# WPI-MMR/gym_solo

Measured on AMD Instinct MI355X. Metric: env-steps/s (whole node), 4096 Solo8 envs/GPU, 1/2/4/8 MI355X, higher is better.
Workload: dtype f64

## Files before the change

### gym_solo_amd/csrc/solo_engine.hip

```cpp
#include <hip/hip_runtime.h>

#include <cstdio>
#include <cstdlib>
#include <cstring>
#include <new>
#include <string>
#include <vector>

#include "solo_wave_ops.h"
#include "solo_pgs_gfx950.h"
#include "solo_step_kernel.h"
#include "solo_launch.h"

namespace solo_engine_detail {

struct EngineBase {
  virtual ~EngineBase() {}
  virtual int set_program(const SoloProgram* p) = 0;
  virtual int reset(const uint8_t* mask, hipStream_t s) = 0;
  virtual int settle(hipStream_t s) = 0;
  virtual int set_targets(const void* a, hipStream_t s) = 0;
  virtual int step(const void* a, uint32_t flags, hipStream_t s) = 0;
  virtual int rollout(const void* a, int k, uint32_t flags, void* obs_out, void* reward_out, void* done_out, hipStream_t s) = 0;
  virtual int view(SoloStateView* v) = 0;
  virtual int set_params(int which, const void* p, hipStream_t s) = 0;
  virtual int set_terrain(const SoloTerrain* t, hipStream_t s) = 0;
  virtual int set_order(const int32_t* order, hipStream_t s) = 0;
  virtual int time_step(const void* a, uint32_t flags, int reps, hipStream_t s, double* ms) = 0;
  virtual int time_rollout(const void* a, int k, uint32_t flags, void* obs_out, void* reward_out, void* done_out, hipStream_t s, double* ms) = 0;
  virtual int plan(int k, SoloLaunchPlan* out) = 0;
  virtual int reserve(int k, uint32_t flags) = 0;
  virtual int check_fault() = 0;
  virtual const char* kernel_name() = 0;
  virtual int set_control(const SoloControl* c, hipStream_t s) = 0;
  virtual int get_control(SoloControl* out) = 0;
  virtual int set_contact_sensing(int32_t enable, hipStream_t s) = 0;
  virtual int get_contacts(void** out) = 0;
  std::string err;
};

#define HIP_TRY(expr)                                                                 \
  do {                                                                                \
    hipError_t e_ = (expr);                                                           \
    if (e_ != hipSuccess) {                                                           \
      err = std::string(#expr) + ": " + hipGetErrorString(e_);                        \
      return SOLO_ERR_HIP;                                                            \
    }                                                                                 \
  } while (0)

constexpr size_t kStatsBytes = (size_t)SOLO_STATS_SHARDS * SOLO_STATS_WIDTH * sizeof(double);

template <typename T>
struct Engine final : EngineBase {
  SoloConfig cfg;
  SoloModel model;
  int n = 0, device = 0, obs_dim = 0;
  bool have_program = false;
  SoloControl control{};
  bool settling = false;
  solo::KParams<T> hparams;
  solo::KParams<T>* dparams = nullptr;
  T *state = nullptr, *snapshot = nullptr, *targets = nullptr, *params = nullptr, *obs = nullptr,
    *reward = nullptr, *settle_actions = nullptr, *warm = nullptr;
  T* traj = nullptr;
  uint8_t* done = nullptr;
  int32_t* term_count = nullptr;
  int32_t *order = nullptr, *cost = nullptr;
  bool use_order = false;
  double* stats = nullptr;
  T* terrain = nullptr;
  int32_t* queue = nullptr;
  size_t queue_ints = 0;
  int traj_steps = 0;
  int32_t* fault_host = nullptr;
  int32_t* fault_dev = nullptr;
  bool sensing = false;
  T *contact = nullptr, *contact_traj = nullptr;
#ifdef SOLO_STAMPS
  unsigned long long* stamps = nullptr;
#endif

  ~Engine() override {
    (void)hipSetDevice(device);
    for (int g = 0; g < kMaxStreams; ++g) {
      if (sub[g]) (void)hipStreamDestroy(sub[g]);
      if (ev_join[g]) (void)hipEventDestroy(ev_join[g]);
    }
    if (ev_fork) (void)hipEventDestroy(ev_fork);
    for (void* p : {(void*)dparams, (void*)state, (void*)snapshot, (void*)targets, (void*)params,
                    (void*)obs, (void*)reward, (void*)settle_actions, (void*)done,
                    (void*)term_count, (void*)order, (void*)cost, (void*)stats, (void*)terrain, (void*)traj, (void*)queue, (void*)warm, (void*)contact, (void*)contact_traj})
// ... 630 lines not shown
```

### gym_solo_amd/csrc/solo_step_kernel.h

```cpp
#pragma once

#include "solo_kernel_params.h"
#include "solo_outputs.h"

#if defined(SOLO_STAMPS) && defined(SOLO_STAMPS_LIGHT)
#define SOLO_STAMP(B, i)                                                                          \
  do {                                                                                            \
    if (((i) == 0 || (i) == 14) && solo::lane_id() == 0)                                          \
      (B).stamps[(size_t)(B).stamp_row * 32 + (i)] = __builtin_amdgcn_s_memrealtime();         \
  } while (0)
#elif defined(SOLO_STAMPS)
#ifdef SOLO_STAMPS_EPILOGUE
#define SOLO_STAMP_ON(i) ((i) == 0 || (i) >= 13)
#define SOLO_STAMP_E(B, i) SOLO_STAMP_AT(B, i)
#else
#define SOLO_STAMP_ON(i) true
#endif
#define SOLO_STAMP(B, i) do { if (SOLO_STAMP_ON(i)) SOLO_STAMP_AT(B, i); } while (0)
#define SOLO_STAMP_AT(B, i)                                                                       \
  do {                                                                                            \
    if (solo::lane_id() == 0) {                                                                   \
      const unsigned long long t_ = __builtin_amdgcn_s_memtime();                                 \
      (B).stamps[(size_t)(B).stamp_row * 32 + (i)] = t_;                                            \
      (B).acc[(i)] += t_ - (B).acc[16];                                                           \
      (B).acc[16] = t_;                                                                           \
    }                                                                                             \
  } while (0)
#else
#define SOLO_STAMP(B, i) do {} while (0)
#endif
#ifndef SOLO_STAMP_E
#define SOLO_STAMP_E(B, i) do {} while (0)
#endif

#ifndef SOLO_PGS_SWEEP_HOOK
#define SOLO_PGS_SWEEP_HOOK(it, pend, lam, v) do {} while (0)
#endif

namespace solo {

template <typename T> struct V3 { T x, y, z; };
template <typename T> __device__ __forceinline__ V3<T> operator+(V3<T> a, V3<T> b) { return {a.x + b.x, a.y + b.y, a.z + b.z}; }
template <typename T> __device__ __forceinline__ V3<T> operator-(V3<T> a, V3<T> b) { return {a.x - b.x, a.y - b.y, a.z - b.z}; }
template <typename T> __device__ __forceinline__ V3<T> operator*(T s, V3<T> a) { return {s * a.x, s * a.y, s * a.z}; }
template <typename T> __device__ __forceinline__ T dot(V3<T> a, V3<T> b) { return a.x * b.x + a.y * b.y + a.z * b.z; }
template <typename T> __device__ __forceinline__ V3<T> cross(V3<T> a, V3<T> b) {
  return {a.y * b.z - a.z * b.y, a.z * b.x - a.x * b.z, a.x * b.y - a.y * b.x};
}
template <typename T> __device__ __forceinline__ V3<T> roty(T c, T s, V3<T> v) {
  return {c * v.x + s * v.z, v.y, c * v.z - s * v.x};
}
template <typename T> __device__ __forceinline__ V3<T> ycross(V3<T> r) { return {r.z, T(0), -r.x}; }
template <typename T> __device__ __forceinline__ V3<T> symmul(const T* I, V3<T> v) {
  return {I[0] * v.x + I[3] * v.y + I[4] * v.z, I[3] * v.x + I[1] * v.y + I[5] * v.z,
          I[4] * v.x + I[5] * v.y + I[2] * v.z};
}
template <typename T> __device__ __forceinline__ void rot_inertia_y(T c, T s, const T* I, T* o) {
  const T cc = c * c, ss = s * s, cs = c * s;
  o[0] = cc * I[0] + T(2) * cs * I[4] + ss * I[2];
  o[1] = I[1];
  o[2] = ss * I[0] - T(2) * cs * I[4] + cc * I[2];
  o[3] = c * I[3] + s * I[5];
  o[4] = cs * (I[2] - I[0]) + (cc - ss) * I[4];
  o[5] = c * I[5] - s * I[3];
}
template <typename T> __device__ __forceinline__ T sum_over_group16(T x) { return wave_sum_group16(x); }
template <typename T> __device__ __forceinline__ V3<T> select(bool p, V3<T> a, V3<T> b) { return {p ? a.x : b.x, p ? a.y : b.y, p ? a.z : b.z}; }
template <typename T> __device__ __forceinline__ T both_halves(T x) { return x + wave_other_half16(x); }
template <typename T> __device__ __forceinline__ V3<T> both_halves(V3<T> v) { return {both_halves(v.x), both_halves(v.y), both_halves(v.z)}; }
template <typename T> __device__ __forceinline__ T from_lower(T x) { return wave_from_lower_half16(x); }
template <typename T> __device__ __forceinline__ V3<T> from_lower(V3<T> v) { return {from_lower(v.x), from_lower(v.y), from_lower(v.z)}; }


}
namespace solo {
#ifndef SOLO_PRIO_SWEEPS_F64
#define SOLO_PRIO_SWEEPS_F64 12
#endif
#ifndef SOLO_QUEUE_SPINS
#define SOLO_QUEUE_SPINS (1 << 22)
#endif
#ifndef SOLO_PRIO_BY_ROWS
#define SOLO_PRIO_BY_ROWS 1
#endif
#ifndef SOLO_PRIO_ROWS_1
#define SOLO_PRIO_ROWS_1 11
#define SOLO_PRIO_ROWS_2 17
#define SOLO_PRIO_ROWS_3 23
#endif
__device__ __forceinline__ int priority_by_rows(int rows) { return rows > SOLO_PRIO_ROWS_3 ? 3 : (rows > SOLO_PRIO_ROWS_2 ? 2 : (rows > SOLO_PRIO_ROWS_1 ? 1 : 0)); }
template <typename T> constexpr int kPrioSweeps = sizeof(T) == 4 ? 8 : SOLO_PRIO_SWEEPS_F64;
#ifndef SOLO_F64_WAVES
#define SOLO_F64_WAVES 4
#endif
template <typename T> constexpr int kRowBlockReals = sizeof(T) == 4 ? 64 * 8 + 64 * 8 : (SOLO_F64_WAVES >= 4 ? 800 : 896);
#ifndef SOLO_W4_PIPELINED_BUILD
#define SOLO_W4_PIPELINED_BUILD 0
#endif
#ifndef SOLO_W4_HYBRID_BUILD
#define SOLO_W4_HYBRID_BUILD 1
#endif
constexpr int kLegSlots = 26;

template <typename T> struct RowView {
  int type, body;
  const T* geo;
};
template <typename T> struct StepTables {
  const LegConst<T>* legc;
  const int32_t* rowtype;
  const T (*rowgeo)[4];
  __device__ __forceinline__ RowView<T> row(int lane) const {
    const int tb = rowtype[lane];
    return {tb & 15, (tb >> 4) & 15, rowgeo[(tb >> 8) & 255]};
  }
};

constexpr unsigned long long kPhaseLanes[3] = {0xc003c003c003c003ull,
                                               0x0924092409240924ull,
                                               0x36d836d836d836d8ull};

template <typename T, bool kResid, bool kFromLds>
__device__ __forceinline__ int pgs_solve_cpp(const ColumnBank<T>& A, T& v, T& lamv, T& cand, T& dl, unsigned long long& pend, T& lo, T& hi,
                                             T tol_rel, int lane, T mu, bool is_tan1, bool is_tangent, unsigned long long ph0,
                                             unsigned long long ph1, unsigned long long ph2, int iters, T diag, T resid_thr, int& n_changed) {
  using R = Real<T>;
  int it = 0;
#pragma unroll 1
  for (; it < iters && pend != 0ull; ++it) {
    const T lam_sweep_start = lamv;
    bool normals_moved = false;
#pragma unroll
    for (int phase = 0; phase < 3; ++phase) {
      const unsigned long long phase_lanes = phase == 0 ? ph0 : (phase == 1 ? ph1 : ph2);
      if (phase == 2 && normals_moved) {
        T n1, n2;
        if constexpr (ColumnBank<T>::kCompact) { n1 = wave_slot_below<1>(lamv); n2 = wave_slot_below<2>(lamv); }
        else { n1 = wave_lane_below<1>(lamv); n2 = wave_lane_below<2>(lamv); }
        const T lim = mu * (is_tan1 ? n1 : n2);
        lo = is_tangent ? -lim : lo;
        hi = is_tangent ? lim : hi;
        cand = R::clamp(v, lo, hi);
        dl = cand - lamv;
        pend = wave_ballot(R::abs(dl) > R::abs(lamv) * tol_rel);
      }
      if ((pend & phase_lanes) == 0ull) continue;
      if (phase == 1) normals_moved = true;
#pragma unroll
      for (int bank = 0; bank < (kFromLds ? 1 : ColumnBank<T>::kBanks); ++bank) {
        unsigned long long window = kFromLds ? phase_lanes : (phase_lanes & ColumnBank<T>::bank_lanes(bank));
#pragma unroll 1
        while ((pend & window) != 0ull) {
          const int r = __builtin_ctzll(pend & window);
          window &= ~((2ull << r) - 1ull);
          const T col = kFromLds ? A.column(r) : A.get(bank, r);
          const T delta = wave_readlane(dl, r);
          v = R::fma(col, delta, v);
          lamv = (lane == r) ? cand : lamv;
          cand = R::clamp(v, lo, hi);
          dl = cand - lamv;
          pend = wave_ballot(R::abs(dl) > R::abs(lamv) * tol_rel);
          ++n_changed;
        }
      }
    }
    SOLO_PGS_SWEEP_HOOK(it, pend, lamv, v);
    const T dvel = (lamv - lam_sweep_start) * diag;
    if (kResid && wave_ballot(dvel * dvel > resid_thr) == 0ull) { ++it; break; }
  }
  return it;
}

template <typename T, bool kResid, bool kPipelinedBuild, bool kCtl = false, bool kContact = false, typename FetchTarget>
__device__ __forceinline__ T physics_solve(const StepConst<T>& C, const KBuffers<T>& B, const StepTables<T>& tabs,
                                           const T* s_state, T my_target, FetchTarget&& fetch_target, T* s_rowvec, T (*s_hext)[8], unsigned char* s_rowleg,
                                           T* s_keep, T (*s_leg)[kLegSlots], const T* s_math, T mu, T mass_scale, int lane, int& row_at, bool& target_bad,
                                           int& prio_sweeps, int& prio_steps, int& prio_rot, T warm_in = T(0), bool warm_on = false,
                                           const CtlConst<T>* ctl = nullptr, T* s_cnrm = nullptr) {
  constexpr bool kCompact = ColumnBank<T>::kCompact;
  constexpr int kRS = ColumnBank<T>::kRowStride;
// ... 369 lines not shown
    hh[0] = jl1 * s_leg[leg][12];
    hh[1] = (jl2 - s_leg[leg][13] * hh[0]) * s_leg[leg][14];
  }
  T w = jl1 * s_leg[leg][15] + jl2 * s_leg[leg][16] - bias;
#pragma unroll
  for (int i = 0; i < 6; ++i) w += jb[i] * s_keep[21 + i];
  T diag = hh[0] * hh[0] + hh[1] * hh[1];
#pragma unroll
  for (int i = 0; i < 6; ++i) diag += gh[i] * gh[i];
  T inv_d = R::rcp(diag);
  if (!live) {
#pragma unroll
    for (int i = 0; i < 6; ++i) gh[i] = T(0);
    hh[0] = hh[1] = T(0);
    inv_d = T(0);
    w = T(0);
    diag = T(0);
  }
  T lam0 = T(0);
  if constexpr (kResid) {
    if (warm_on) {
      if constexpr (sizeof(T) == 8) mu = s_keep[27];
      const T imp0 = C.motor_impulse;
      lam0 = live ? C.warm_factor * warm_in : T(0);
      if (is_motor) lam0 = R::clamp(lam0, -imp0, imp0);
      else if (type == ROW_NORMAL || is_limit) lam0 = R::max(lam0, T(0));
      const T wn1 = wave_lane_below<1>(lam0), wn2 = wave_lane_below<2>(lam0);
      if (type == ROW_TAN1 || type == ROW_TAN2) {
        const T lim0 = (rc.body == BODY_BASE ? s_keep[29] : mu) * (type == ROW_TAN1 ? wn1 : wn2);
        lam0 = R::clamp(lam0, -lim0, lim0);
      }
      if (!live) lam0 = T(0);
      T zz[6], yy[2];
#pragma unroll
      for (int i = 0; i < 6; ++i) zz[i] = gh[i] * lam0;
      yy[0] = hh[0] * lam0;
      yy[1] = hh[1] * lam0;
      wave_reduce_rows(zz, yy);
      T alam = hh[0] * yy[0] + hh[1] * yy[1];
#pragma unroll
      for (int i = 0; i < 6; ++i) alam += gh[i] * zz[i];
      w += alam;
    }
  }
  const unsigned long long touching = wave_ballot(live && type == ROW_NORMAL);
  const unsigned long long limited = wave_ballot(live && is_limit);
  int sv_type = live ? type : (int)ROW_IDLE;
  T sv_v0 = w * -inv_d + lam0, sv_nid = -inv_d, sv_diag = diag;
  T sv_lam0 = lam0;
  T sv_imp = ctl_imp;
  T sg[6], sh[2];
  int sv_leg = leg, n_live = 64;
  bool sv_on_base = rc.body == BODY_BASE;
  if constexpr (!kCompact) {
#pragma unroll
    for (int i = 0; i < 6; ++i) { s_rowvec[lane * kRS + i] = gh[i]; sg[i] = gh[i]; }
    s_rowvec[lane * kRS + 6] = hh[0];
    s_rowvec[lane * kRS + 7] = hh[1];
    sh[0] = hh[0]; sh[1] = hh[1];
    s_hext[lane][2 * leg] = hh[0];
    s_hext[lane][2 * leg + 1] = hh[1];
    row_at = lane;
    wave_sync();
  } else {
    const unsigned long long live_lanes = wave_ballot(live);
    n_live = __builtin_popcountll(live_lanes);
    const int below = wave_count_below(live_lanes);
    const int dst = live ? below : n_live + (lane - below);
    row_at = dst;
#pragma unroll
    for (int i = 0; i < 6; ++i) s_rowvec[dst * kRS + i] = gh[i];
    s_rowvec[dst * kRS + 6] = hh[0];
    s_rowvec[dst * kRS + 7] = hh[1];
    s_rowleg[dst] = (unsigned char)leg;
    const int tl = wave_push_int(sv_type | (leg << 4) | (sv_on_base ? 64 : 0), dst);
    sv_v0 = wave_push(sv_v0, dst);
    sv_nid = wave_push(sv_nid, dst);
    if constexpr (kResid) { sv_diag = wave_push(sv_diag, dst); if (warm_on) sv_lam0 = wave_push(sv_lam0, dst); }
    if constexpr (kCtl) sv_imp = wave_push(sv_imp, dst);
    sv_type = tl & 15;
    sv_leg = (tl >> 4) & 3;
    sv_on_base = (tl & 64) != 0;
    wave_sync();
#pragma unroll
    for (int i = 0; i < 6; ++i) sg[i] = s_rowvec[lane * kRS + i];
    sh[0] = s_rowvec[lane * kRS + 6];
    sh[1] = s_rowvec[lane * kRS + 7];
  }

  SOLO_STAMP(B, 7);
#if SOLO_PRIO_BY_ROWS
  {
    const int rows_now = kCompact ? n_live : __builtin_popcountll(wave_ballot(live));
    wave_set_priority_level(prio_sweeps > kPrioSweeps<T> * prio_steps ? 3 : priority_by_rows(rows_now));
  }
#endif
  ColumnBank<T> A;
  if constexpr (kCompact) A.init(sg, sh, sv_nid, lane, s_rowvec, s_rowleg, sv_leg);
  else A.init(sg, sh, sv_nid, lane, s_rowvec, &s_hext[0][2 * sv_leg]);
  const bool overflow = kCompact && n_live > ColumnBank<T>::kSlots;
  if constexpr (!kCompact) {
#pragma unroll
    for (int l2 = 0; l2 < 4; ++l2) {
#pragma unroll
      for (int kk = 0; kk < 2; ++kk) A.build(16 * l2 + kk);
    }
    const unsigned touching_lo = (unsigned)touching, touching_hi = (unsigned)(touching >> 32);
    if (limited != 0ull) {
#pragma unroll
      for (int l2 = 0; l2 < 4; ++l2) {
#pragma unroll
        for (int kk = 14; kk < 16; ++kk)
          if ((limited >> (16 * l2 + kk)) & 1ull) A.build(16 * l2 + kk);
      }
    }
#pragma unroll
    for (int l2 = 0; l2 < 4; ++l2) {
#pragma unroll
      for (int j = 0; j < 4; ++j) {
        const int r0 = 16 * l2 + 2 + 3 * j;
        if (((r0 < 32 ? touching_lo : touching_hi) >> (r0 & 31)) & 1u) {
#pragma unroll
          for (int q = 0; q < 3; ++q) A.build(r0 + q);
        }
      }
    }
  } else if (!overflow) {
    if constexpr (SOLO_F64_WAVES >= 4 && SOLO_W4_HYBRID_BUILD && kPipelinedBuild) {
      typename ColumnBank<T>::Row cur = A.fetch(0);
      {
        typename ColumnBank<T>::Row nxt = A.fetch(1);
        A.build_from(0, cur);
        cur = A.fetch(2);
        A.build_from(1, nxt);
      }
#pragma unroll
      for (int j = 2; j < ColumnBank<T>::kSlots; j += 3) {
        if (n_live > j) {
          if (j + 2 < 17) {
            typename ColumnBank<T>::Row nxt = A.fetch(j + 1);
            A.build_from(j, cur);
            cur = A.fetch(j + 2);
            A.build_from(j + 1, nxt);
            nxt = A.fetch(j + 3);
            A.build_from(j + 2, cur);
            cur = nxt;
          } else {
            if (j == 17) A.build_from(j, cur); else A.build(j);
            if (j + 1 < ColumnBank<T>::kSlots) A.build(j + 1);
            if (j + 2 < ColumnBank<T>::kSlots) A.build(j + 2);
          }
        }
      }
    } else if constexpr (SOLO_F64_WAVES >= 4 && !SOLO_W4_PIPELINED_BUILD) {
      A.build(0); A.build(1);
#pragma unroll
      for (int j = 2; j < ColumnBank<T>::kSlots; j += 3) {
        if (n_live > j) {
          A.build(j);
          if (j + 1 < ColumnBank<T>::kSlots) A.build(j + 1);
          if (j + 2 < ColumnBank<T>::kSlots) A.build(j + 2);
        }
      }
    } else {
    typename ColumnBank<T>::Row cur = A.fetch(0);
    {
      const typename ColumnBank<T>::Row n1 = A.fetch(1);
      A.build_from(0, cur);
      cur = A.fetch(2);
      A.build_from(1, n1);
    }
#pragma unroll
    for (int j = 2; j < ColumnBank<T>::kSlots; j += 3) {
      if (n_live > j) {
        const typename ColumnBank<T>::Row n1 = A.fetch(j + 1 < 64 ? j + 1 : 63);
        A.build_from(j, cur);
        if (j + 1 < ColumnBank<T>::kSlots) {
          const typename ColumnBank<T>::Row n2 = A.fetch(j + 2 < 64 ? j + 2 : 63);
          A.build_from(j + 1, n1);
          cur = A.fetch(j + 3 < 64 ? j + 3 : 63);
          if (j + 2 < ColumnBank<T>::kSlots) A.build_from(j + 2, n2);
        }
      }
    }
    }
  }
  (void)touching; (void)limited;
  SOLO_STAMP(B, 8);
  const bool sv_motor = sv_type == ROW_MOTOR, sv_limit = sv_type == ROW_LIMIT, sv_normal = sv_type == ROW_NORMAL;
  const bool is_tan1 = sv_type == ROW_TAN1, is_tangent = sv_type == ROW_TAN1 || sv_type == ROW_TAN2;
  const T imp = C.motor_impulse;
  if constexpr (sizeof(T) == 8) mu = s_keep[27];
  mu = sv_on_base ? s_keep[29] : mu;
  T lo = T(0), hi = T(0);
  if (sv_motor) { lo = kCtl ? sv_imp : -imp; hi = kCtl ? sv_imp : imp; }
  else if (sv_normal || sv_limit) hi = R::big();
  T lamv = sv_lam0;
  T v = sv_v0;
  if constexpr (kResid) {
    if (warm_on) {
      T n1, n2;
      if constexpr (kCompact) { n1 = wave_slot_below<1>(lamv); n2 = wave_slot_below<2>(lamv); }
      else { n1 = wave_lane_below<1>(lamv); n2 = wave_lane_below<2>(lamv); }
      const T lim = mu * (is_tan1 ? n1 : n2);
      lo = is_tangent ? -lim : lo;
      hi = is_tangent ? lim : hi;
    }
  }
  const T tol_rel = T(wave_uniform(C.ulp_tol)) * R::half_ulp();
  const int iters = wave_uniform(C.iterations);
  const T resid_thr = C.resid_thr;
  unsigned long long ph0 = kPhaseLanes[0], ph1 = kPhaseLanes[1], ph2 = kPhaseLanes[2];
  if constexpr (kCompact) {
    ph0 = wave_ballot(sv_motor || sv_limit);
    ph1 = wave_ballot(sv_normal);
    ph2 = wave_ballot(is_tangent);
  }
  T cand = R::clamp(v, lo, hi);
  T dl = cand - lamv;
  unsigned long long pend = wave_ballot(R::abs(dl) > R::abs(lamv) * tol_rel);
  int n_changed = 0;
  int it = 0;
#ifdef SOLO_PGS_GFX950
  if (!overflow) {
    const unsigned long long tan1_lanes = wave_ballot(is_tan1), tangent_lanes = wave_ballot(is_tangent);
    if constexpr (!kResid) {
      it = pgs_solve_gfx950(A, v, lamv, cand, dl, pend, lo, hi, tol_rel, lane, mu, tan1_lanes, tangent_lanes, ph0, ph1, ph2, iters, n_changed);
    } else {
#pragma unroll 1
      for (;;) {
        const T lam_sweep_start = lamv;
        const int n = pgs_solve_gfx950(A, v, lamv, cand, dl, pend, lo, hi, tol_rel, lane, mu, tan1_lanes, tangent_lanes, ph0, ph1, ph2, 1, n_changed);
        it += n;
        if (n == 0 || it >= iters) break;
        const T dvel = (lamv - lam_sweep_start) * sv_diag;
        if (wave_ballot(dvel * dvel > resid_thr) == 0ull) break;
      }
    }
#if defined(SOLO_PGS_HAZARD_PROBE)
    {
      const unsigned stuck = __builtin_amdgcn_s_getreg((0 << 11) | (27 << 6) | 1);
      asm volatile("s_set_gpr_idx_off\n\ts_nop 1");
      if (stuck != 0 && lane == 0) stats_add(&B.stats[7], 1.0);
    }
#endif
  } else
#else
  if (!overflow) it = pgs_solve_cpp<T, kResid, false>(A, v, lamv, cand, dl, pend, lo, hi, tol_rel, lane, mu, is_tan1, is_tangent, ph0, ph1, ph2, iters, sv_diag, resid_thr, n_changed);
  else
#endif
  {
    if constexpr (kCompact) it = pgs_solve_cpp<T, kResid, true>(A, v, lamv, cand, dl, pend, lo, hi, tol_rel, lane, mu, is_tan1, is_tangent, ph0, ph1, ph2, iters, sv_diag, resid_thr, n_changed);
  }
#ifdef SOLO_STAMPS
  if (lane == 0) {
    const unsigned long long hw = (unsigned long long)(__builtin_amdgcn_s_getreg(63492) & 0xfffff), xcc = (unsigned long long)(__builtin_amdgcn_s_getreg(63508) & 0xf);
    B.stamps[(size_t)B.stamp_row * 32 + 15] = (unsigned long long)(it & 0xffff) | ((unsigned long long)__builtin_popcountll(touching) << 16) | (xcc << 24) | (hw << 28) | ((unsigned long long)(n_changed & 0xffff) << 48);
#ifndef SOLO_STAMPS_LIGHT
    B.acc[15] += (unsigned long long)it;
    B.acc[0] += (unsigned long long)n_changed;
#endif
  }
#endif
  (void)n_changed;
  if constexpr (kCompact) lamv = wave_pull(lamv, row_at);
  prio_sweeps += it;
  prio_steps += 1;
  prio_rot = prio_rot == 2 ? 0 : prio_rot + 1;
// ... 170 lines not shown
```

### gym_solo_amd/csrc/solo_wave_ops.h

```cpp
#pragma once

#include <hip/hip_runtime.h>

namespace solo {

__device__ __forceinline__ int lane_id() { return threadIdx.x; }
__device__ __forceinline__ int block_id() { return blockIdx.x; }

__device__ __forceinline__ void wave_sync() { __syncthreads(); }
__device__ __forceinline__ void wave_fence_global() {
  __builtin_amdgcn_fence(__ATOMIC_RELEASE, "workgroup");
  __builtin_amdgcn_fence(__ATOMIC_ACQUIRE, "workgroup");
}
template <typename P> __device__ __forceinline__ P* wave_opaque(P* p) {
  asm volatile("" : "+s"(p));
  return p;
}
__device__ __forceinline__ unsigned long long wave_opaque_bits(unsigned long long x) {
  asm volatile("" : "+s"(x));
  return x;
}
__device__ __forceinline__ int wave_opaque_lane(int lane) {
  asm volatile("" : "+v"(lane));
  return lane;
}
__device__ __forceinline__ int wave_fresh_lane() {
  int lane;
  asm volatile("v_mbcnt_lo_u32_b32 %0, -1, 0\n\tv_mbcnt_hi_u32_b32 %0, -1, %0" : "=v"(lane));
  return lane;
}
__device__ __forceinline__ int wave_readlane_int(int x, int lane) { return __builtin_amdgcn_readlane(x, lane); }
__device__ __forceinline__ int wave_uniform(int x) { return __builtin_amdgcn_readfirstlane(x); }

__device__ __forceinline__ float wave_readlane(float x, int lane) {
  return __int_as_float(__builtin_amdgcn_readlane(__float_as_int(x), lane));
}
__device__ __forceinline__ double wave_readlane(double x, int lane) {
  const long long b = __double_as_longlong(x);
  const int lo = __builtin_amdgcn_readlane((int)(b & 0xffffffffll), lane);
  const int hi = __builtin_amdgcn_readlane((int)(b >> 32), lane);
  return __longlong_as_double(((long long)hi << 32) | (unsigned int)lo);
}
__device__ __forceinline__ float wave_sum_legs(float x) {
  auto a = __builtin_amdgcn_permlane16_swap(__float_as_uint(x), __float_as_uint(x), false, false);
  const float s = __uint_as_float(a[0]) + __uint_as_float(a[1]);
  auto b = __builtin_amdgcn_permlane32_swap(__float_as_uint(s), __float_as_uint(s), false, false);
  return __uint_as_float(b[0]) + __uint_as_float(b[1]);
}
__device__ __forceinline__ double wave_sum_legs(double x) {
  unsigned lo = (unsigned)(__double_as_longlong(x) & 0xffffffffll), hi = (unsigned)(__double_as_longlong(x) >> 32);
  auto a = __builtin_amdgcn_permlane16_swap(lo, lo, false, false);
  auto b = __builtin_amdgcn_permlane16_swap(hi, hi, false, false);
  const double s = __longlong_as_double(((long long)a[0] & 0xffffffffll) | ((long long)b[0] << 32)) +
                   __longlong_as_double(((long long)a[1] & 0xffffffffll) | ((long long)b[1] << 32));
  lo = (unsigned)(__double_as_longlong(s) & 0xffffffffll); hi = (unsigned)(__double_as_longlong(s) >> 32);
  auto c = __builtin_amdgcn_permlane32_swap(lo, lo, false, false);
  auto d = __builtin_amdgcn_permlane32_swap(hi, hi, false, false);
  return __longlong_as_double(((long long)c[0] & 0xffffffffll) | ((long long)d[0] << 32)) +
         __longlong_as_double(((long long)c[1] & 0xffffffffll) | ((long long)d[1] << 32));
}
template <int CTRL> __device__ __forceinline__ float dpp_mov(float x) {
  return __int_as_float(__builtin_amdgcn_update_dpp(0, __float_as_int(x), CTRL, 0xf, 0xf, true));
}
template <int CTRL> __device__ __forceinline__ double dpp_mov(double x) {
  const long long b = __double_as_longlong(x);
  const int lo = __builtin_amdgcn_update_dpp(0, (int)(b & 0xffffffffll), CTRL, 0xf, 0xf, false);
  const int hi = __builtin_amdgcn_update_dpp(0, (int)(b >> 32), CTRL, 0xf, 0xf, false);
  return __longlong_as_double(((long long)hi << 32) | (unsigned int)lo);
}
template <typename T> __device__ __forceinline__ T wave_other_half16(T x) { return dpp_mov<0x128>(x); }
template <int BANKS> __device__ __forceinline__ float dpp_half_bcast(float x) {
  return __int_as_float(__builtin_amdgcn_update_dpp(__float_as_int(x), __float_as_int(x), 0x128, 0xf, BANKS, false));
}
template <int BANKS> __device__ __forceinline__ double dpp_half_bcast(double x) {
  const long long b = __double_as_longlong(x);
  const int lo = __builtin_amdgcn_update_dpp((int)(b & 0xffffffffll), (int)(b & 0xffffffffll), 0x128, 0xf, BANKS, false);
  const int hi = __builtin_amdgcn_update_dpp((int)(b >> 32), (int)(b >> 32), 0x128, 0xf, BANKS, false);
  return __longlong_as_double(((long long)hi << 32) | (unsigned int)lo);
}
template <typename T> __device__ __forceinline__ T wave_from_lower_half16(T x) { return dpp_half_bcast<0x3>(x); }
template <typename T> __device__ __forceinline__ T wave_from_upper_half16(T x) { return dpp_half_bcast<0xc>(x); }
template <int N, typename T> __device__ __forceinline__ T wave_lane_below(T x) { return dpp_mov<0x110 + N>(x); }
template <int N, typename T> __device__ __forceinline__ T wave_slot_below(T x) {
#pragma unroll
  for (int i = 0; i < N; ++i) x = dpp_mov<0x138>(x);
  return x;
}
__device__ __forceinline__ int wave_count_below(unsigned long long mask) {
  return (int)__builtin_amdgcn_mbcnt_hi((unsigned)(mask >> 32), __builtin_amdgcn_mbcnt_lo((unsigned)mask, 0u));
}
__device__ __forceinline__ int wave_push_int(int x, int dst) { return __builtin_amdgcn_ds_permute(dst << 2, x); }
__device__ __forceinline__ float wave_push(float x, int dst) { return __int_as_float(__builtin_amdgcn_ds_permute(dst << 2, __float_as_int(x))); }
__device__ __forceinline__ double wave_push(double x, int dst) {
  const long long b = __double_as_longlong(x);
  const int lo = __builtin_amdgcn_ds_permute(dst << 2, (int)(b & 0xffffffffll));
  const int hi = __builtin_amdgcn_ds_permute(dst << 2, (int)(b >> 32));
  return __longlong_as_double(((long long)hi << 32) | (unsigned int)lo);
}
__device__ __forceinline__ float wave_pull(float x, int src) { return __int_as_float(__builtin_amdgcn_ds_bpermute(src << 2, __float_as_int(x))); }
__device__ __forceinline__ double wave_pull(double x, int src) {
  const long long b = __double_as_longlong(x);
  const int lo = __builtin_amdgcn_ds_bpermute(src << 2, (int)(b & 0xffffffffll));
  const int hi = __builtin_amdgcn_ds_bpermute(src << 2, (int)(b >> 32));
  return __longlong_as_double(((long long)hi << 32) | (unsigned int)lo);
}
template <typename T> __device__ __forceinline__ T wave_sum_group16(T x) {
  x += dpp_mov<0x128>(x);
  x += dpp_mov<0x124>(x);
  x += dpp_mov<0x122>(x);
  x += dpp_mov<0x121>(x);
  return x;
}
__device__ __forceinline__ float wave_sum_all(float x) {
  x = wave_sum_group16(x);
  asm("s_nop 1\n\tv_add_f32_dpp %0, %0, %0 row_bcast:15 row_mask:0xa bank_mask:0xf\n\t"
      "s_nop 1\n\tv_add_f32_dpp %0, %0, %0 row_bcast:31 row_mask:0xc bank_mask:0xf" : "+v"(x));
  return wave_readlane(x, 63);
}
__device__ __forceinline__ double wave_sum_all(double x) { return wave_sum_legs(wave_sum_group16(x)); }
__device__ __forceinline__ unsigned long long wave_ballot(bool p) { return __ballot(p); }

__device__ __forceinline__ void wave_reduce_rows(float (&z)[6], float (&y)[2]) {
#define SOLO_DPP_STAGE8(CTRL)                                                                      \
  "v_add_f32_dpp %0, %0, %0 " CTRL " row_mask:0xf bank_mask:0xf\n\t"                                \
  "v_add_f32_dpp %1, %1, %1 " CTRL " row_mask:0xf bank_mask:0xf\n\t"                                \
  "v_add_f32_dpp %2, %2, %2 " CTRL " row_mask:0xf bank_mask:0xf\n\t"                                \
  "v_add_f32_dpp %3, %3, %3 " CTRL " row_mask:0xf bank_mask:0xf\n\t"                                \
  "v_add_f32_dpp %4, %4, %4 " CTRL " row_mask:0xf bank_mask:0xf\n\t"                                \
  "v_add_f32_dpp %5, %5, %5 " CTRL " row_mask:0xf bank_mask:0xf\n\t"                                \
  "v_add_f32_dpp %6, %6, %6 " CTRL " row_mask:0xf bank_mask:0xf\n\t"                                \
  "v_add_f32_dpp %7, %7, %7 " CTRL " row_mask:0xf bank_mask:0xf\n\t"
#define SOLO_DPP_STAGE6(CTRL, MASK)                                                                \
  "v_add_f32_dpp %0, %0, %0 " CTRL " row_mask:" MASK " bank_mask:0xf\n\t"                           \
  "v_add_f32_dpp %1, %1, %1 " CTRL " row_mask:" MASK " bank_mask:0xf\n\t"                           \
  "v_add_f32_dpp %2, %2, %2 " CTRL " row_mask:" MASK " bank_mask:0xf\n\t"                           \
  "v_add_f32_dpp %3, %3, %3 " CTRL " row_mask:" MASK " bank_mask:0xf\n\t"                           \
  "v_add_f32_dpp %4, %4, %4 " CTRL " row_mask:" MASK " bank_mask:0xf\n\t"                           \
  "v_add_f32_dpp %5, %5, %5 " CTRL " row_mask:" MASK " bank_mask:0xf\n\t"
  asm("s_nop 1\n\t"
      SOLO_DPP_STAGE8("row_ror:8") SOLO_DPP_STAGE8("row_ror:4") SOLO_DPP_STAGE8("row_ror:2") SOLO_DPP_STAGE8("row_ror:1")
      SOLO_DPP_STAGE6("row_bcast:15", "0xa") SOLO_DPP_STAGE6("row_bcast:31", "0xc")
      : "+v"(z[0]), "+v"(z[1]), "+v"(z[2]), "+v"(z[3]), "+v"(z[4]), "+v"(z[5]), "+v"(y[0]), "+v"(y[1]));
// ... 49 lines not shown
  __device__ __forceinline__ T dot(const T* rg, const T* rh, T same) const {
    const T a1 = __builtin_fma(g[2], rg[2], __builtin_fma(g[1], rg[1], g[0] * rg[0]));
    const T a2 = __builtin_fma(g[5], rg[5], __builtin_fma(g[4], rg[4], g[3] * rg[3]));
    return __builtin_fma(same, __builtin_fma(h[1], rh[1], h[0] * rh[0]), a1 + a2);
  }
};
template <> struct RowDot<float> {
  solo_f32x2 g01, g23, g45, h01;
  __device__ __forceinline__ void set(const float* gh, const float* hh) {
    g01 = solo_f32x2{gh[0], gh[1]}; g23 = solo_f32x2{gh[2], gh[3]}; g45 = solo_f32x2{gh[4], gh[5]};
    h01 = solo_f32x2{hh[0], hh[1]};
  }
  __device__ __forceinline__ float dot(const float* rg, const float* rh) const {
    const solo_f32x2* r = reinterpret_cast<const solo_f32x2*>(rg);
    solo_f32x2 acc = g01 * r[0];
    acc = g23 * r[1] + acc;
    acc = g45 * r[2] + acc;
    acc = h01 * *reinterpret_cast<const solo_f32x2*>(rh) + acc;
    return acc.x + acc.y;
  }
};

typedef float solo_f32x32 __attribute__((ext_vector_type(32)));
template <typename T> struct ColumnBank;
template <> struct ColumnBank<float> {
  static constexpr bool kResident = true;
  static constexpr bool kCompact = false;
  static constexpr int kSlots = 64, kRowStride = 8;
  static constexpr int kBanks = 2;
  static __device__ __forceinline__ constexpr unsigned long long bank_lanes(int b) { return 0xffffffffull << (32 * b); }
  RowDot<float> own;
  float nid;
  int lane;
  const float* rowvec;
  const float* hext;
  solo_f32x32 a0, a1;
  __device__ __forceinline__ void init(const float* gh, const float* hh, float nid_, int lane_, const float* rowvec_, const float* hext_) {
    own.set(gh, hh); nid = nid_; lane = lane_; rowvec = rowvec_; hext = hext_;
  }
  __device__ __forceinline__ float column(int r) const { const float m = (lane == r) ? 0.0f : nid; return m * own.dot(rowvec + 8 * r, hext + 8 * r); }
  __device__ __forceinline__ void build(int r) { const float x = column(r); if (r < 32) a0[r] = x; else a1[r - 32] = x; }
  __device__ __forceinline__ float get(int bank, int r) const { return bank == 0 ? a0[r & 31] : a1[r & 31]; }
};
typedef double solo_f64x16 __attribute__((ext_vector_type(16)));
template <> struct ColumnBank<double> {
  static constexpr bool kResident = true;
  static constexpr bool kCompact = true;
  static constexpr int kSlots = 32, kRowStride = 8;
  static constexpr int kBanks = 2;
  static __device__ __forceinline__ constexpr unsigned long long bank_lanes(int b) { return 0xffffull << (16 * b); }
  RowDot<double> own;
  double nid;
  int lane;
  const double* rowvec;
  const unsigned char* rowleg;
  int leg;
  solo_f64x16 a0, a1;
  __device__ __forceinline__ void init(const double* gh, const double* hh, double nid_, int lane_, const double* rowvec_, const unsigned char* rowleg_, int leg_) {
    own.set(gh, hh); nid = nid_; lane = lane_; rowvec = rowvec_; rowleg = rowleg_; leg = leg_;
  }
  __device__ __forceinline__ double same_leg(int leg_r) const { return leg_r == leg ? 1.0 : 0.0; }
  __device__ __forceinline__ double column(int r) const {
    const double m = (lane == r) ? 0.0 : nid;
    return m * own.dot(rowvec + kRowStride * r, rowvec + kRowStride * r + 6, same_leg(rowleg[r]));
  }
  __device__ __forceinline__ void build(int r) {
    const double x = column(r);
    if (r < 16) a0[r] = x; else a1[r - 16] = x;
  }
  struct Row { double g[6], h[2]; int leg; };
  __device__ __forceinline__ Row fetch(int r) const {
    Row x;
#pragma unroll
    for (int i = 0; i < 6; ++i) x.g[i] = rowvec[kRowStride * r + i];
    x.h[0] = rowvec[kRowStride * r + 6]; x.h[1] = rowvec[kRowStride * r + 7];
    x.leg = rowleg[r];
    return x;
  }
  __device__ __forceinline__ void build_from(int r, const Row& x) {
    const double m = (lane == r) ? 0.0 : nid;
    const double c = m * own.dot(x.g, x.h, same_leg(x.leg));
    if (r < 16) a0[r] = c; else a1[r - 16] = c;
  }
  __device__ __forceinline__ double get(int bank, int r) const { return bank == 0 ? a0[r & 15] : a1[r & 15]; }
};

template <typename B> using ColdArgs = const __attribute__((address_space(4))) B*;
template <typename B> __device__ __forceinline__ ColdArgs<B> wave_cold_args(const B& by_value) {
  (void)by_value;
  auto base = (const __attribute__((address_space(4))) char*)__builtin_amdgcn_kernarg_segment_ptr();
  ColdArgs<B> p = (ColdArgs<B>)(base + sizeof(void*));
  asm volatile("" : "+s"(p));
  return p;
}

__device__ __forceinline__ int wave_atomic_add(int32_t* p, int v) { return __hip_atomic_fetch_add(p, v, __ATOMIC_RELAXED, __HIP_MEMORY_SCOPE_AGENT); }
__device__ __forceinline__ int wave_atomic_load(const int32_t* p) { return __hip_atomic_load(p, __ATOMIC_RELAXED, __HIP_MEMORY_SCOPE_AGENT); }
__device__ __forceinline__ void wave_atomic_store(int32_t* p, int v) { __hip_atomic_store(p, v, __ATOMIC_RELAXED, __HIP_MEMORY_SCOPE_AGENT); }
__device__ __forceinline__ float wave_load_shared(const float* p) { return __uint_as_float(__hip_atomic_load(reinterpret_cast<const unsigned*>(p), __ATOMIC_RELAXED, __HIP_MEMORY_SCOPE_AGENT)); }
__device__ __forceinline__ double wave_load_shared(const double* p) { return __longlong_as_double((long long)__hip_atomic_load(reinterpret_cast<const unsigned long long*>(p), __ATOMIC_RELAXED, __HIP_MEMORY_SCOPE_AGENT)); }
__device__ __forceinline__ void wave_store_shared(float* p, float v) { __hip_atomic_store(reinterpret_cast<unsigned*>(p), __float_as_uint(v), __ATOMIC_RELAXED, __HIP_MEMORY_SCOPE_AGENT); }
__device__ __forceinline__ void wave_store_shared(double* p, double v) { __hip_atomic_store(reinterpret_cast<unsigned long long*>(p), (unsigned long long)__double_as_longlong(v), __ATOMIC_RELAXED, __HIP_MEMORY_SCOPE_AGENT); }
__device__ __forceinline__ void wave_release_device() {
  __builtin_amdgcn_fence(__ATOMIC_RELEASE, "workgroup");
  asm volatile("s_waitcnt vmcnt(0)" ::: "memory");
}
__device__ __forceinline__ void wave_acquire_device() { __builtin_amdgcn_fence(__ATOMIC_ACQUIRE, "workgroup"); }
__device__ __forceinline__ void wave_backoff() { __builtin_amdgcn_s_sleep(8); }
__device__ __forceinline__ void wave_fault_set(int32_t* p) { __hip_atomic_store(p, 1, __ATOMIC_RELAXED, __HIP_MEMORY_SCOPE_SYSTEM); }
__device__ __forceinline__ int wave_xcc_id() { return (int)(__builtin_amdgcn_s_getreg((3 << 11) | 20) & 0xf); }

__device__ __forceinline__ int wave_slot_id() { return (int)(__builtin_amdgcn_s_getreg(((4 - 1) << 11) | 4) & 0xf); }
__device__ __forceinline__ void wave_set_priority_level(int p) {
  if (p >= 3) __builtin_amdgcn_s_setprio(3);
  else if (p == 2) __builtin_amdgcn_s_setprio(2);
  else if (p == 1) __builtin_amdgcn_s_setprio(1);
  else __builtin_amdgcn_s_setprio(0);
}

template <typename T> struct Real;
template <> struct Real<float> {
  static __device__ __forceinline__ float sqrt(float x) { return __builtin_amdgcn_sqrtf(x); }
  static __device__ __forceinline__ float rsqrt(float x) { return __builtin_amdgcn_rsqf(x); }
  static __device__ __forceinline__ float rcp(float x) { return __builtin_amdgcn_rcpf(x); }
  static constexpr int kTabSize = 0;
  static __device__ __forceinline__ void sincos(float x, float* s, float* c, const float* = nullptr) {
    const float k = __builtin_rintf(x * 0.63661977236758134f);
    float r = __builtin_fmaf(k, -1.57079601287841796875f, x);
    r = __builtin_fmaf(k, -3.1391647326017846e-07f, r);
    r = __builtin_fmaf(k, -5.3903029534742385e-15f, r);
    const float r2 = r * r;
    float sp = __builtin_fmaf(r2, -1.9515295891e-4f, 8.3321608736e-3f);
    sp = __builtin_fmaf(r2, sp, -1.6666654611e-1f);
    const float sn = __builtin_fmaf(r2 * r, sp, r);
    float cp = __builtin_fmaf(r2, 2.443315711809948e-5f, -1.388731625493765e-3f);
    cp = __builtin_fmaf(r2, cp, 4.166664568298827e-2f);
    const float cs = __builtin_fmaf(r2 * r2, cp, __builtin_fmaf(r2, -0.5f, 1.0f));
    const int q = (int)k;
    const float a = (q & 1) ? cs : sn, b = (q & 1) ? sn : cs;
    *s = (q & 2) ? -a : a;
    *c = ((q + 1) & 2) ? -b : b;
  }
  static __device__ __forceinline__ void sinc_cos(float x2, float* sinc, float* c, const float* = nullptr) {
    if (__builtin_expect(__builtin_amdgcn_readfirstlane(__float_as_int(x2)) > 0x3d800000, 0)) {
      const float x = __builtin_amdgcn_sqrtf(x2);
      float sn, cs;
      sincos(x, &sn, &cs);
      *sinc = sn * __builtin_amdgcn_rcpf(x);
      *c = cs;
      return;
    }
    float sp = __builtin_fmaf(x2, -1.9841270e-4f, 8.3333333e-3f);
    sp = __builtin_fmaf(x2, sp, -1.6666667e-1f);
    *sinc = __builtin_fmaf(x2, sp, 1.0f);
    float cp = __builtin_fmaf(x2, 2.4801587e-5f, -1.3888889e-3f);
    cp = __builtin_fmaf(x2, cp, 4.1666667e-2f);
    cp = __builtin_fmaf(x2, cp, -0.5f);
    *c = __builtin_fmaf(x2, cp, 1.0f);
  }
  static __device__ __forceinline__ float atan2(float y, float x) {
    const float ax = fabsf(x), ay = fabsf(y);
    const float mx = fmaxf(ax, ay), mn = fminf(ax, ay);
    const float a = (mx == 0.0f) ? 0.0f : mn * __builtin_amdgcn_rcpf(mx);
    const float s2 = a * a;
    float p = __builtin_fmaf(s2, -0.0040545654f, 0.021862952f);
    p = __builtin_fmaf(s2, p, -0.05591232f);
// ... 139 lines not shown
```

Before: 190.8 million.

## Build f64 column bank two rows at a time using both wave halves

When the live contact rows fit in the column bank, each 32-lane half of the wave now computes a different row's dot products. The two results are exchanged with permlane32_swap, so each build step fills two column entries. Lanes in the upper half take over the lower half's row data (nid, leg and own row vector), so both halves cover the same 32 rows. The aim is to halve the number of serial f64 dot-product steps in the build phase. The cost is extra cross-lane swaps and a replacement of the pipelined fetch/build schedule. Correctness depends on live rows being at most 32 and on the upper half's lanes holding no needed state.

```diff
diff --git a/gym_solo_amd/csrc/solo_engine.hip b/gym_solo_amd/csrc/solo_engine.hip
--- a/gym_solo_amd/csrc/solo_engine.hip
+++ b/gym_solo_amd/csrc/solo_engine.hip
@@ -7,6 +7,9 @@
 #include <string>
 #include <vector>
 
+#ifndef SOLO_F64_PAIR_BUILD
+#define SOLO_F64_PAIR_BUILD 1
+#endif
 #include "solo_wave_ops.h"
 #include "solo_pgs_gfx950.h"
 #include "solo_step_kernel.h"
diff --git a/gym_solo_amd/csrc/solo_step_kernel.h b/gym_solo_amd/csrc/solo_step_kernel.h
--- a/gym_solo_amd/csrc/solo_step_kernel.h
+++ b/gym_solo_amd/csrc/solo_step_kernel.h
@@ -96,6 +96,9 @@
 template <typename T> constexpr int kRowBlockReals = sizeof(T) == 4 ? 64 * 8 + 64 * 8 : (SOLO_F64_WAVES >= 4 ? 800 : 896);
 #ifndef SOLO_W4_PIPELINED_BUILD
 #define SOLO_W4_PIPELINED_BUILD 0
+#endif
+#ifndef SOLO_F64_PAIR_BUILD
+#define SOLO_F64_PAIR_BUILD 0
 #endif
 #ifndef SOLO_W4_HYBRID_BUILD
 #define SOLO_W4_HYBRID_BUILD 1
@@ -631,10 +634,18 @@
     sv_leg = (tl >> 4) & 3;
     sv_on_base = (tl & 64) != 0;
     wave_sync();
-#pragma unroll
-    for (int i = 0; i < 6; ++i) sg[i] = s_rowvec[lane * kRS + i];
-    sh[0] = s_rowvec[lane * kRS + 6];
-    sh[1] = s_rowvec[lane * kRS + 7];
+    int own_slot = lane;
+#if SOLO_F64_PAIR_BUILD
+    if (n_live <= ColumnBank<T>::kSlots) {
+      own_slot = lane & 31;
+      sv_nid = wave_from_lower_half32(sv_nid);
+      sv_leg = (wave_from_lower_half32(tl) >> 4) & 3;
+    }
+#endif
+#pragma unroll
+    for (int i = 0; i < 6; ++i) sg[i] = s_rowvec[own_slot * kRS + i];
+    sh[0] = s_rowvec[own_slot * kRS + 6];
+    sh[1] = s_rowvec[own_slot * kRS + 7];
   }
 
   SOLO_STAMP(B, 7);
@@ -675,6 +686,16 @@
       }
     }
   } else if (!overflow) {
+#if SOLO_F64_PAIR_BUILD
+    A.build_pair(0);
+#pragma unroll
+    for (int j = 2; j < ColumnBank<T>::kSlots; j += 3) {
+      if (n_live > j) {
+        if (j % 2 == 0) { A.build_pair(j); A.build_pair(j + 2); }
+        else A.build_pair(j + 1);
+      }
+    }
+#else
     if constexpr (SOLO_F64_WAVES >= 4 && SOLO_W4_HYBRID_BUILD && kPipelinedBuild) {
       typename ColumnBank<T>::Row cur = A.fetch(0);
       {
@@ -733,6 +754,7 @@
       }
     }
     }
+#endif
   }
   (void)touching; (void)limited;
   SOLO_STAMP(B, 8);
diff --git a/gym_solo_amd/csrc/solo_wave_ops.h b/gym_solo_amd/csrc/solo_wave_ops.h
--- a/gym_solo_amd/csrc/solo_wave_ops.h
+++ b/gym_solo_amd/csrc/solo_wave_ops.h
@@ -1,6 +1,10 @@
 #pragma once
 
 #include <hip/hip_runtime.h>
+
+#ifndef SOLO_F64_PAIR_BUILD
+#define SOLO_F64_PAIR_BUILD 0
+#endif
 
 namespace solo {
 
@@ -58,6 +62,16 @@
   auto d = __builtin_amdgcn_permlane32_swap(hi, hi, false, false);
   return __longlong_as_double(((long long)c[0] & 0xffffffffll) | ((long long)d[0] << 32)) +
          __longlong_as_double(((long long)c[1] & 0xffffffffll) | ((long long)d[1] << 32));
+}
+__device__ __forceinline__ int wave_from_lower_half32(int x) {
+  auto a = __builtin_amdgcn_permlane32_swap((unsigned)x, (unsigned)x, false, false);
+  return (int)a[0];
+}
+__device__ __forceinline__ double wave_from_lower_half32(double x) {
+  const unsigned lo = (unsigned)(__double_as_longlong(x) & 0xffffffffll), hi = (unsigned)(__double_as_longlong(x) >> 32);
+  auto a = __builtin_amdgcn_permlane32_swap(lo, lo, false, false);
+  auto b = __builtin_amdgcn_permlane32_swap(hi, hi, false, false);
+  return __longlong_as_double(((long long)a[0] & 0xffffffffll) | ((long long)b[0] << 32));
 }
 template <int CTRL> __device__ __forceinline__ float dpp_mov(float x) {
   return __int_as_float(__builtin_amdgcn_update_dpp(0, __float_as_int(x), CTRL, 0xf, 0xf, true));
@@ -273,6 +287,21 @@
     const double c = m * own.dot(x.g, x.h, same_leg(x.leg));
     if (r < 16) a0[r] = c; else a1[r - 16] = c;
   }
+#if SOLO_F64_PAIR_BUILD
+  __device__ __forceinline__ void build_pair(int r) {
+    const int half = lane >> 5;
+    const double* row = rowvec + kRowStride * half;
+    const double m = ((lane & 31) == r + half) ? 0.0 : nid;
+    const double x = m * own.dot(row + kRowStride * r, row + kRowStride * r + 6, same_leg((rowleg + half)[r]));
+    const unsigned lo = (unsigned)(__double_as_longlong(x) & 0xffffffffll), hi = (unsigned)(__double_as_longlong(x) >> 32);
+    auto a = __builtin_amdgcn_permlane32_swap(lo, lo, false, false);
+    auto b = __builtin_amdgcn_permlane32_swap(hi, hi, false, false);
+    const double c0 = __longlong_as_double(((long long)a[0] & 0xffffffffll) | ((long long)b[0] << 32));
+    const double c1 = __longlong_as_double(((long long)a[1] & 0xffffffffll) | ((long long)b[1] << 32));
+    if (r < 16) a0[r] = c0; else a1[r - 16] = c0;
+    if (r + 1 < 16) a0[r + 1] = c1; else a1[r + 1 - 16] = c1;
+  }
+#endif
   __device__ __forceinline__ double get(int bank, int r) const { return bank == 0 ? a0[r & 15] : a1[r & 15]; }
 };
 
```

Measured after the change: 200.9 million (median of 6 runs). 5.3% higher.
